# zhouzypaul/fql

Hardware: AMD Instinct MI355X
Metric: FQL gradient-steps/s (batch=256) (higher is better)
Workload: dtype f32

## Files before the change

### fql_amd/csrc/fql_engine.hip

```cpp
#include "../../include/fql_amd.h"
#include "fql_kernels.h"
#include "fql_conv.h"
#include "fql_chain.h"
#include "fql_aux.h"
#include "fql_ifql.h"
#include "fql_rebrac.h"
#include "fql_sac.h"
#include "fql_bc.h"
#include "fql_iql.h"
#include "fql_iqld.h"
#include "fql_cfgrl.h"
#include <hip/hip_ext.h>
#include "fql_aql.h"

#include <algorithm>
#include <cmath>
#include <cstdarg>
#include <cstdio>
#include <cstdlib>
#include <cstring>
#include <map>
#include <memory>
#include <random>
#include <string>
// ... 145 lines not shown
    EulerFinishArgs ef;
    ConvArgs conv;
    PoolArgs pool;
    PoolBwdArgs poolb;
    ConvWgradArgs cw;
    ConvWredArgs cwr;
    EncDzArgs edz;
    ChainArgs chain;
    const ConvWprepTask* wprep_tasks = nullptr;
    int wprep_n = 0;
    int cw_grid = 0;
    int adam_c0 = 0, adam_n = -1;
    int adam_c1 = 0, adam_n1 = 0;
    int adam_polyak = -1;
    float adam_lr = 0.f;
    DevState* adam_st = nullptr;
    bool adam_fin = false;
    int fin_mode = 0;
    Bound k;
    int level = 0;
    int lane = 0;
    std::vector<int> deps;
};

struct Launch {
    OpType type;
    int grid = 0, ntasks = 0;
    size_t lds = 0;
    void* table = nullptr;
    Op op;
    bool pool_fused = false;
    int lane = 0;
    bool tmt2 = false, kbig = false, euler = false;
    double macs = 0.0;
    void *table_w = nullptr, *table_l = nullptr, *table_m = nullptr;
    int n_w = 0, n_l = 0, tile_w = 0, tile_l = 0, tile_m = 0;
    std::vector<GemmTask> dg_tasks;
    std::vector<GemmTask> h_gemm;
    std::vector<WgradTask> h_wgrad;
    std::vector<LnBwdTask> h_ln;
    std::vector<MiscTask> h_misc;
    std::shared_ptr<const SideArgs> ka_side;
    std::vector<int> waits;
    bool record_after = false;
    hipEvent_t ev = nullptr;
};

inline bool ka_tasks_env() {
    const char* e = getenv("FQL_KERNARG_TASKS");
    return !e || atoi(e) != 0;
}
inline bool fused_tail_env() {
    const char* e = getenv("FQL_FUSED_TAIL");
    return !e || atoi(e) != 0;
}
inline std::shared_ptr<const SideArgs> ka_side_args(const Launch& L) {
    const size_t ng = L.h_gemm.size(), nw = L.h_wgrad.size(), nl = L.h_ln.size(), nm = L.h_misc.size();
    if (ng > FQL_KA_GEMM || nw > FQL_KA_WGRAD || nl > FQL_KA_LN || nm > FQL_KA_MISC) return nullptr;
    auto a = std::make_shared<SideArgs>();
    std::memset(a.get(), 0, sizeof(SideArgs));
    SideFront& f = a->f;
    f.tile_w = L.tile_w; f.tile_l = L.tile_l; f.tile_m = L.tile_m; f.tl = -1;
    for (int& v : f.g0) v = FQL_KA_FRONT_PAD;
    for (int& v : f.w0) v = FQL_KA_FRONT_PAD;
    for (int& v : f.l0) v = FQL_KA_FRONT_PAD;
    for (size_t i = 0; i < ng; ++i) { a->g[i] = L.h_gemm[i]; if (i) f.g0[i - 1] = L.h_gemm[i].tile0; }
    for (size_t i = 0; i < nw; ++i) { a->w[i] = L.h_wgrad[i]; if (i) f.w0[i - 1] = L.h_wgrad[i].tile0; }
    for (size_t i = 0; i < nl; ++i) { a->l[i] = L.h_ln[i]; if (i) f.l0[i - 1] = L.h_ln[i].tile0; }
    for (size_t i = 0; i < nm; ++i) a->m[i] = L.h_misc[i];
    return a;
}
struct Program {
    std::vector<Op> ops;
    std::vector<Launch> launches;
    bool lane_used[FQL_LANES] = {};
    hipEvent_t ev_fork = nullptr, ev_join[FQL_LANES] = {};
    hipGraph_t graph = nullptr;
    hipGraphExec_t exec = nullptr;
    int64_t macs = 0;
    AqlProgram aql;
    bool aql_tried = false;
};

template <typename P, typename IssueFn>
void issue_lanes(P& pr, hipStream_t s0, const hipStream_t* ls, bool fork, IssueFn&& issue) {
    auto lazy = [](hipEvent_t& e) { if (!e) HIP_CHECK(hipEventCreateWithFlags(&e, hipEventDisableTiming)); };
    bool side = false;
// ... 210 lines not shown
    size_t n_train = 0, n_total = 0, critic_size = 0;
    float *P = nullptr, *G = nullptr, *Mu = nullptr, *Nu = nullptr;
    std::vector<Leaf> leaves;
    int n_train_leaves = 0;
    AdamChunk* d_chunks = nullptr;
    float* d_partials = nullptr;
    int* d_leaf_range = nullptr;
    int n_chunks = 0;

    DevState* d_state = nullptr;
    SrcDesc* d_src = nullptr;
    SrcDesc h_src_shadow{};
    bool src_valid = false;
    SrcDesc* h_src_ring = nullptr;
    int src_ring_pos = 0;

    int B = 0;
    std::vector<void*> ws_allocs;
    float *in_obs = nullptr, *in_act = nullptr, *in_rew = nullptr, *in_mask = nullptr, *in_nobs = nullptr, *in_nact = nullptr;
    float* in_noise[5] = {nullptr, nullptr, nullptr, nullptr, nullptr};
    int64_t* in_idx = nullptr;
    float *X_os = nullptr, *X_bc = nullptr, *X_eu = nullptr, *X_c1 = nullptr, *X_c2 = nullptr, *X_ct = nullptr;
    float *vel = nullptr, *w_rew = nullptr, *w_mask = nullptr, *w_act = nullptr, *tgt = nullptr;
    float *X_e0 = nullptr, *C0 = nullptr, *Abuf[2] = {nullptr, nullptr}, *Vpart = nullptr;
    bool fused_euler = false;
    bool use_chain = false;
    int fill_lane_full = 1;
    std::vector<float*> wf_bc;
    float *wf_w0 = nullptr, *wf_w4 = nullptr;
    WfragTask* d_wfrag = nullptr;
    int wfrag_n = 0, wfrag_grid = 0;
    const bool ka_tasks = ka_tasks_env();
    const bool fused_tail = fused_tail_env();
    unsigned* d_ticket = nullptr;
    std::vector<void*> chain_allocs;
    bool split_build = false;
    bool wide_tiles = false;
    bool split_ok = false;
    int vp_tiles = 0;
    int num_cus = 0;
    PassBuf p_os, p_os_bwd, p_bc, p_eu, p_c1[2], p_c2[2], p_ct[2];
    Program prog_fwdbwd, prog_opt, prog_loss;
    Program prog_opt_split;
    Program prog_full;
    int mod_chunk0[3] = {0, 0, 0}, mod_chunkn[3] = {0, 0, 0};
    Program prog_split;
    hipGraphExec_t split_exec[4] = {nullptr, nullptr, nullptr, nullptr};
    hipGraph_t split_graph[4] = {nullptr, nullptr, nullptr, nullptr};
    hipEvent_t ev_a = nullptr, ev_b = nullptr, ev_c = nullptr;
    bool split_begun = false;
    bool began = false;
    AqlRuntime aql;
    std::vector<AqlDispatch>* aql_rec = nullptr;
    bool last_update_aql = false;
    bool hip_dirty = true;
    void aql_drain() {
        if (!aql.up) return;
        try { aql.drain(); } catch (const AqlError& e) { throw HipError{e.msg}; }
    }

    float *ds_obs = nullptr, *ds_act = nullptr, *ds_rew = nullptr, *ds_mask = nullptr, *ds_nobs = nullptr;
    float* ds_row = nullptr;
    int64_t ds_size = 0, ds_cap = 0, ds_ptr = 0;
    unsigned char *ds_frames = nullptr, *ds_next_frames = nullptr;
    int64_t* ds_init = nullptr;
    int ds_fs = 0;
// ... 1395 lines not shown
                    for (const Op* o : sel) {
                        Launch L;
                        L.type = (OpType)ty;
                        L.op = *o;
                        L.lane = lane;
                        launch_of[o - pr.ops.data()] = (int)pr.launches.size();
                        pr.launches.push_back(L);
                    }
                    continue;
                }
                Launch L;
                L.type = OP_GEMM;
                L.lane = lane;
                for (const Op* o : sel) launch_of[o - pr.ops.data()] = (int)pr.launches.size();
                L.ntasks = (int)sel.size();
                int tile = 0;
                std::vector<GemmTask> tb;
                for (const Op* o : sel) {
                    GemmTask t = o->gemm;
                    t.wk = (t.N <= 16) ? 4 : 2;
                    t.tmt = 1;
                    t.ntn = (t.N / 16 + (4 / t.wk) - 1) / (4 / t.wk);
                    t.tile0 = tile;
                    tile += (t.M / 16) * t.ntn;
                    if (t.K > 512) L.kbig = true;
                    if (t.flags & (GF_A_EULER0 | GF_HEAD_PART | GF_A_LOSSACT)) L.euler = true;
                    L.lds = std::max(L.lds, ((size_t)16 * (t.K + 4) + 1024 + 1280) * sizeof(float));
                    tb.push_back(t);
                }
                L.table = dalloc(owner, tb.size() * sizeof(GemmTask) / sizeof(float) + 4);
                HIP_CHECK(hipMemcpy(L.table, tb.data(), tb.size() * sizeof(GemmTask), hipMemcpyHostToDevice));
                L.grid = tile;
                L.h_gemm = tb;
                pr.launches.push_back(L);
            }
          }
        }
        auto dump_program = [&]() {
            int cnt[FQL_LANES] = {};
            for (const Launch& L : pr.launches) {
                cnt[L.lane]++;
                int lv = -1;
                for (int oi = 0; oi < (int)pr.ops.size(); ++oi) if (launch_of[oi] == (int)(&L - pr.launches.data())) lv = pr.ops[oi].level;
                fprintf(stderr, "[fql] #%2d level %3d lane %d type %2d ntasks %2d grid %5d waits[", (int)(&L - pr.launches.data()), lv, L.lane, (int)L.type, L.ntasks, L.grid);
                for (int w : L.waits) fprintf(stderr, "%d ", w);
                fprintf(stderr, "] :");
                for (int oi = 0; oi < (int)pr.ops.size(); ++oi) {
                    if (launch_of[oi] != (int)(&L - pr.launches.data())) continue;
                    const Op& o = pr.ops[oi];
                    if (o.type == OP_GEMM || o.type == OP_GEMM64) fprintf(stderr, " g%s(%dx%dx%d%s)", o.type == OP_GEMM64 ? "64" : "16", o.gemm.M, o.gemm.N, o.gemm.K, (o.gemm.flags & GF_TRANS_B) ? "T" : "");
                    else if (o.type == OP_WGRAD) fprintf(stderr, " w(%dx%dx%d)", o.wgrad.M, o.wgrad.Kin, o.wgrad.N);
                    else if (o.type == OP_LNBWD) fprintf(stderr, " ln(%d)", o.ln.M);
                    else fprintf(stderr, " t%d", (int)o.type);
                }
                fprintf(stderr, "\n");
            }
            fprintf(stderr, "[fql] launches per lane:");
            for (int l = 0; l < FQL_LANES; ++l) fprintf(stderr, " %d", cnt[l]);
            fprintf(stderr, "\n");
        };
        for (int oi = 0; oi < (int)pr.ops.size(); ++oi) {
            const Op& o = pr.ops[oi];
            const int li = launch_of[oi];
            if (li < 0) continue;
            double m = 0.0;
            if (o.type == OP_GEMM || o.type == OP_GEMM64 || o.type == OP_HEAD_DGRAD) m = (double)o.gemm.M * o.gemm.N * o.gemm.K;
// ... 50 lines not shown
            if (cost < best) { best = cost; xg = gm; }
        }
        return xg;
    }

    hipEvent_t prof_a = nullptr, prof_b = nullptr;
    template <typename... Pm, typename... A>
    void aql_record(void (*k)(Pm...), dim3 g, dim3 b, size_t l, A&&... a) {
        AqlDispatch d;
        d.fn = (const void*)k;
        d.grid[0] = g.x; d.grid[1] = g.y; d.grid[2] = g.z;
        d.block[0] = b.x; d.block[1] = b.y; d.block[2] = b.z;
        d.lds = (uint32_t)l;
        size_t off = 0;
        auto put = [&](auto v) {
            using T = decltype(v);
            off = (off + alignof(T) - 1) & ~(alignof(T) - 1);
            d.args.resize(off + sizeof(T));
            std::memcpy(d.args.data() + off, &v, sizeof(T));
            off += sizeof(T);
        };
        (put(static_cast<Pm>(a)), ...);
        aql_rec->push_back(std::move(d));
    }
#define FQL_LAUNCH(k, g, b, l, st, ...)                                                          \
    do {                                                                                          \
        if (aql_rec) aql_record(k, g, b, (size_t)(l), __VA_ARGS__);                               \
        else if (prof_a) hipExtLaunchKernelGGL(k, g, b, (std::uint32_t)(l), st, prof_a, prof_b, 0u, __VA_ARGS__); \
        else hipLaunchKernelGGL(k, g, b, l, st, __VA_ARGS__);                                     \
    } while (0)
    void issue(const Launch& L, hipStream_t s, int tl) {
        switch (L.type) {
            case OP_GEMM:
                if (L.euler && L.kbig) FQL_LAUNCH((fql_gemm16_euler_kernel<true>), dim3(L.grid), dim3(FQL_THREADS), L.lds, s, (const GemmTask*)L.table, L.ntasks, tl);
                else if (L.euler) FQL_LAUNCH((fql_gemm16_euler_kernel<false>), dim3(L.grid), dim3(FQL_THREADS), L.lds, s, (const GemmTask*)L.table, L.ntasks, tl);
                else if (L.kbig) FQL_LAUNCH((fql_gemm16_kernel<true>), dim3(L.grid), dim3(FQL_THREADS), L.lds, s, (const GemmTask*)L.table, L.ntasks, tl);
                else FQL_LAUNCH((fql_gemm16_kernel<false>), dim3(L.grid), dim3(FQL_THREADS), L.lds, s, (const GemmTask*)L.table, L.ntasks, tl);
                break;
            case OP_GEMM64:
                if (L.ka_side) {
                    SideArgs a = *L.ka_side; a.f.tl = tl;
                    if (L.tmt2) FQL_LAUNCH(fql_side_big_ka_kernel, dim3(L.grid), dim3(FQL_THREADS), L.lds, s, a);
                    else if (cfg.precision == 2) FQL_LAUNCH(fql_side_split_ka_kernel, dim3(L.grid), dim3(FQL_THREADS), L.lds, s, a);
                    else FQL_LAUNCH(fql_side_ka_kernel, dim3(L.grid), dim3(FQL_THREADS), L.lds, s, a);
                }
                else if (L.tmt2)
                    FQL_LAUNCH(fql_side_big_kernel, dim3(L.grid), dim3(FQL_THREADS), L.lds, s, (const GemmTask*)L.table, L.ntasks,
                                       (const WgradTask*)L.table_w, L.n_w, (const LnBwdTask*)L.table_l, L.n_l, L.tile_w, L.tile_l,
                                       (const MiscTask*)L.table_m, L.tile_m, tl);
                else if (cfg.precision == 2)
                    FQL_LAUNCH(fql_side_split_kernel, dim3(L.grid), dim3(FQL_THREADS), L.lds, s, (const GemmTask*)L.table, L.ntasks,
                                       (const WgradTask*)L.table_w, L.n_w, (const LnBwdTask*)L.table_l, L.n_l, L.tile_w, L.tile_l,
                                       (const MiscTask*)L.table_m, L.tile_m, tl);
                else
                    FQL_LAUNCH(fql_side_kernel, dim3(L.grid), dim3(FQL_THREADS), L.lds, s, (const GemmTask*)L.table, L.ntasks,
                                       (const WgradTask*)L.table_w, L.n_w, (const LnBwdTask*)L.table_l, L.n_l, L.tile_w, L.tile_l,
                                       (const MiscTask*)L.table_m, L.tile_m, tl);
                break;
            case OP_PREP:
                { PrepArgs pa = L.op.prep; pa.tl = tl; FQL_LAUNCH(fql_prep_kernel, dim3((pa.B + 3) / 4), dim3(FQL_THREADS), 0, s, pa); }
                break;
            case OP_EULER_FIN:
                FQL_LAUNCH(fql_euler_finish_kernel, dim3((L.op.ef.M * L.op.ef.ad + FQL_THREADS - 1) / FQL_THREADS), dim3(FQL_THREADS), 0, s, L.op.ef);
                break;
            case OP_LOSS_ACTOR:
                FQL_LAUNCH(fql_loss_actor_kernel, dim3(1), dim3(FQL_THREADS), 0, s, L.op.la);
                break;
// ... 3833 lines not shown
        const int si = code / 100, k = code % 100;
        EncBuf::St& s = b->st[si];
        if (k == 50) {
            const EncStack& st = h->encs[enc].stacks[si];
            std::vector<int32_t> plan{st.conv[0].pool_fused ? 1 : 0};
            for (size_t j = 0; j < st.conv.size(); ++j) {
                const ConvL& c = st.conv[j];
                const int H = j == 0 ? st.H : st.H / 2, W = j == 0 ? st.W : st.W / 2, Ci = pad16c(c.cin);
                const bool u8 = si == 0 && j == 0;
                plan.push_back(u8 ? (h->cfg.precision == 2 ? 1 : 0) : (c.split ? 1 : 0));
                plan.push_back(fql_engine::conv_rows(H, W, Ci, c.cout, false));
                plan.push_back(u8 ? 0 : fql_engine::conv_rows(H, W, c.cout, Ci, false));
                plan.push_back(fql_engine::conv_rows(H, W, Ci, c.cout, true, u8));
            }
            if (bytes > plan.size() * sizeof(int32_t)) return FQL_E_INVALID;
            std::memcpy(out, plan.data(), bytes);
            return FQL_OK;
        }
        if (k == 0) src = s.c0;
        else if (k == 1) src = s.pool;
        else if (k == 4) src = s.arg;
        else if (k % 10 == 2 && (size_t)(k / 10) < s.c1.size()) src = s.c1[k / 10];
        else if (k % 10 == 3 && (size_t)(k / 10) < s.y.size()) src = s.y[k / 10];
    }
    if (!src) return FQL_E_NOTFOUND;
    auto it = b->bytes.find(src);
    if (it == b->bytes.end() || bytes > it->second) return FQL_E_INVALID;
    hipDeviceSynchronize();
    return hipMemcpy(out, src, bytes, hipMemcpyDeviceToHost) == hipSuccess ? FQL_OK : FQL_E_HIP;
}

namespace {
enum { PLAN_K_OTHER = 0, PLAN_K_GEMM16, PLAN_K_GEMM16_KBIG, PLAN_K_GEMM16_EULER, PLAN_K_GEMM16_EULER_KBIG, PLAN_K_SIDE, PLAN_K_SIDE_SPLIT, PLAN_K_SIDE_BIG,
       PLAN_K_CHAIN, PLAN_K_CHAIN_SPLIT };
struct PlanKernel { const void* fn; int entry, H, V; };
template <typename... Pm> const void* plan_fn(void (*k)(Pm...)) { return (const void*)k; }
const std::vector<PlanKernel>& plan_kernels() {
#define FQL_PLAN_CHAIN(HH) \
    {plan_fn(fql_chain_kernel<HH, 0>), PLAN_K_CHAIN, HH, 0}, {plan_fn(fql_chain_kernel<HH, 1>), PLAN_K_CHAIN, HH, 1},                    \
    {plan_fn(fql_chain_kernel<HH, 2>), PLAN_K_CHAIN, HH, 2}, {plan_fn(fql_chain_kernel<HH, 3>), PLAN_K_CHAIN, HH, 3},                    \
    {plan_fn(fql_chain_split_kernel<HH, 0>), PLAN_K_CHAIN_SPLIT, HH, 0}, {plan_fn(fql_chain_split_kernel<HH, 1>), PLAN_K_CHAIN_SPLIT, HH, 1}, \
    {plan_fn(fql_chain_split_kernel<HH, 2>), PLAN_K_CHAIN_SPLIT, HH, 2}
    static const std::vector<PlanKernel> t = {
        {plan_fn(fql_gemm16_kernel<false>), PLAN_K_GEMM16, 0, 0}, {plan_fn(fql_gemm16_kernel<true>), PLAN_K_GEMM16_KBIG, 0, 0},
        {plan_fn(fql_gemm16_euler_kernel<false>), PLAN_K_GEMM16_EULER, 0, 0}, {plan_fn(fql_gemm16_euler_kernel<true>), PLAN_K_GEMM16_EULER_KBIG, 0, 0},
        {plan_fn(fql_side_kernel), PLAN_K_SIDE, 0, 0}, {plan_fn(fql_side_split_kernel), PLAN_K_SIDE_SPLIT, 0, 0},
        {plan_fn(fql_side_big_kernel), PLAN_K_SIDE_BIG, 0, 0}, FQL_PLAN_CHAIN(256), FQL_PLAN_CHAIN(512),
        {plan_fn(fql_side_ka_kernel), PLAN_K_SIDE, 0, 0}, {plan_fn(fql_side_split_ka_kernel), PLAN_K_SIDE_SPLIT, 0, 0},
        {plan_fn(fql_side_big_ka_kernel), PLAN_K_SIDE_BIG, 0, 0}};
#undef FQL_PLAN_CHAIN
    return t;
}
}
extern "C" int fql_debug_plan(fql_handle h, void* out, size_t bytes) {
    if (!h || (bytes && !out) || bytes % sizeof(int32_t)) return FQL_E_INVALID;
    if (h->visual || !h->prog_full.exec || h->prog_full.launches.empty()) return FQL_E_STATE;
    try {
        const Program& pr = h->prog_full;
        const std::vector<AqlDispatch> rec = h->record_dispatches(pr);
        std::vector<int32_t> plan{0, (int32_t)pr.launches.size()};
        for (size_t i = 0; i < pr.launches.size(); ++i) {
            const Launch& L = pr.launches[i];
            const AqlDispatch& d = rec[i];
            PlanKernel k{d.fn, PLAN_K_OTHER, 0, 0};
            for (const PlanKernel& c : plan_kernels()) if (c.fn == d.fn) k = c;
            const bool table = L.type == OP_GEMM || L.type == OP_GEMM64;
            const bool chain = L.type == OP_CHAIN;
            if (chain != (k.entry == PLAN_K_CHAIN || k.entry == PLAN_K_CHAIN_SPLIT)) throw HipError{"internal: a chain launch records an unknown kernel"};
            if (table == (k.entry == PLAN_K_OTHER || chain)) throw HipError{"internal: a GEMM launch records an unknown kernel"};
            plan.insert(plan.end(), {(int32_t)i, L.lane, (int32_t)L.type, (int32_t)(d.grid[0] * d.grid[1] * d.grid[2]), k.entry,
                                     table ? (int32_t)L.h_gemm.size() : 0, table ? (int32_t)L.h_wgrad.size() : 0, table ? (int32_t)L.h_ln.size() : 0,
                                     chain ? 1 : 0});
            if (table) {
                for (const GemmTask& t : L.h_gemm) plan.insert(plan.end(), {t.M, t.N, t.K, (L.type == OP_GEMM ? 16 : 32) * t.tmt, t.wk, t.xg});
                for (const WgradTask& t : L.h_wgrad) plan.insert(plan.end(), {t.M, t.Kin, t.N, k.entry == PLAN_K_SIDE_SPLIT ? 1 : 0});
                for (const LnBwdTask& t : L.h_ln) plan.push_back(t.M);
            }
            if (chain) {
                ChainArgs ca;
                if (d.args.size() < sizeof(ChainArgs)) throw HipError{"internal: a chain launch records no ChainArgs"};
                std::memcpy(&ca, d.args.data(), sizeof(ChainArgs));
                plan.insert(plan.end(), {ca.M, k.H, k.V, ca.xg, k.entry == PLAN_K_CHAIN_SPLIT ? 1 : 0});
// ... 153 lines not shown
            F.ev = nullptr; F.waits.clear();
            F.ka_side = nullptr;
            std::vector<WfragTask> h_wf;
            std::vector<const void*> tg, tw, tl, tm;
            std::vector<int> ng, nw, nl, nm, sg, sw, sl, sm;
            int cg = 0, cw = 0, cl = 0, cm = 0, ntot = 0;
            for (int k = 0; k < K; ++k) {
                const Launch& L = m[k]->prog_full.launches[li];
                if (L0.type == OP_WFRAG) {
                    tg.push_back(m[k]->d_wfrag); ng.push_back(m[k]->wfrag_n); sg.push_back(cg); cg += m[k]->wfrag_grid; ntot += m[k]->wfrag_n;
                } else if (L0.type == OP_GEMM64) {
                    tg.push_back(L.table); ng.push_back(L.ntasks); sg.push_back(cg); cg += L.tile_w;
                    tw.push_back(L.table_w); nw.push_back(L.n_w); sw.push_back(cw); cw += L.tile_l - L.tile_w;
                    tl.push_back(L.table_l); nl.push_back(L.n_l); sl.push_back(cl); cl += L.tile_m - L.tile_l;
                    tm.push_back(L.table_m); nm.push_back(L.grid - L.tile_m); sm.push_back(0); cm += L.grid - L.tile_m;
                } else {
                    tg.push_back(L.table); ng.push_back(L.ntasks); sg.push_back(cg); cg += L.grid; ntot += L.ntasks;
                }
            }
            if (L0.type == OP_WFRAG) {
                F.table = fuse<WfragTask>(tg, ng, sg, h_wf); F.ntasks = ntot; F.grid = cg;
            } else if (L0.type == OP_GEMM64) {
                F.table = fuse<GemmTask>(tg, ng, sg, F.h_gemm);
                F.table_w = fuse<WgradTask>(tw, nw, sw, F.h_wgrad);
                F.table_l = fuse<LnBwdTask>(tl, nl, sl, F.h_ln);
                F.table_m = fuse<MiscTask>(tm, nm, sm, F.h_misc, false);
                F.ntasks = F.n_w = F.n_l = 0;
                for (int k = 0; k < K; ++k) { F.ntasks += ng[k]; F.n_w += nw[k]; F.n_l += nl[k]; }
                F.tile_w = cg; F.tile_l = cg + cw; F.tile_m = cg + cw + cl; F.grid = F.tile_m + cm;
                if (m[0]->ka_tasks) F.ka_side = ka_side_args(F);
            } else {
                F.table = fuse<GemmTask>(tg, ng, sg, F.h_gemm);
                F.ntasks = ntot; F.grid = cg;
            }
            G.L = F;
            return G;
        }
        auto it = multi_entries().find(rec[0].fn);
        if (it == multi_entries().end()) invalid("agent groups: launch %d (op type %d) has no multi-instance kernel", li, (int)L0.type);
        std::vector<uint8_t> args;
        for (int k = 0; k < K; ++k) {
            if (rec[k].args.size() != it->second.arg_bytes) invalid("internal: launch %d records %zu argument bytes, its struct has %zu", li, rec[k].args.size(), it->second.arg_bytes);
            args.insert(args.end(), rec[k].args.begin(), rec[k].args.end());
        }
        G.multi = it->second.launch;
        G.grid = dim3(rec[0].grid[0], K);
        G.block = dim3(rec[0].block[0], rec[0].block[1], rec[0].block[2]);
        G.lds = rec[0].lds;
        G.args = upload(args.data(), args.size());
        return G;
    }

    void issue(GLaunch& G, hipStream_t s) {
        if (!G.table) { G.multi(G.grid, G.block, G.lds, s, G.args); return; }
        if (G.L.type == OP_WFRAG) hipLaunchKernelGGL(fql_wfrag_kernel, dim3(G.L.grid), dim3(FQL_THREADS), 0, s, (const WfragTask*)G.L.table, G.L.ntasks, -1);
        else m[0]->issue(G.L, s, -1);
    }

    void capture() {
        capture_graph(lanes[0], [&] { issue_lanes(*this, lanes[0], lanes, true, [&](GLaunch& G, hipStream_t s) { issue(G, s); }); }, graph, exec);
    }

    void release() {
        if (lanes[0]) hipStreamSynchronize(lanes[0]);
        if (last == hipStreamLegacy) hipDeviceSynchronize();
        if (ev_done) hipEventSynchronize(ev_done);
// ... 1 lines not shown
        if (exec) hipGraphExecDestroy(exec);
        if (graph) hipGraphDestroy(graph);
        destroy_lane_events(*this);
        for (hipEvent_t e : {ev_in, ev_done}) if (e) hipEventDestroy(e);
        for (void* p : allocs) hipFree(p);
        if (d_idx) hipFree(d_idx);
        for (hipStream_t s : lanes) if (s) hipStreamDestroy(s);
    }
};

namespace {
void group_check(const fql_handle* members, int k) {
    if (!members || k <= 0) invalid("fql_group_create: members must be a non-empty array (k = %d)", k);
    for (int i = 0; i < k; ++i) {
        fql_handle h = members[i];
        if (!h) invalid("fql_group_create: member %d is NULL", i);
        for (int j = 0; j < i; ++j) if (members[j] == h) invalid("fql_group_create: member %d appears twice", i);
        if (h->group) invalid("fql_group_create: member %d already belongs to a group", i);
        if (h->visual) invalid("fql_group_create: member %d has an encoder (groups take state agents only)", i);
        if (h->cfg.precision != 0) invalid("fql_group_create: member %d has precision %d (groups take fp32 members only)", i, h->cfg.precision);
        if (h->began) invalid("fql_group_create: member %d is between fql_update_begin and fql_update_end", i);
        require_graph(h->prog_full);
        fql_config a = h->cfg, b = members[0]->cfg;
        a.alpha = b.alpha = 0.f;
        a.batch_size = b.batch_size = 0;
        if (std::memcmp(&a, &b, sizeof a) != 0)
            invalid("fql_group_create: member %d's config differs from member 0's in more than seed and alpha", i);
        if (h->B != members[0]->B) invalid("fql_group_create: member %d has batch size %d, member 0 has %d", i, h->B, members[0]->B);
        const Program& p = h->prog_full, &p0 = members[0]->prog_full;
        if (p.launches.size() != p0.launches.size()) invalid("fql_group_create: member %d's update has %zu launches, member 0's %zu", i, p.launches.size(), p0.launches.size());
        for (size_t li = 0; li < p.launches.size(); ++li) {
            const Launch &L = p.launches[li], &L0 = p0.launches[li];
            if (L.type != L0.type || L.lane != L0.lane || L.grid != L0.grid || L.waits != L0.waits || L.tmt2 != L0.tmt2 ||
                L.kbig != L0.kbig || L.euler != L0.euler || L.record_after != L0.record_after || L.lds != L0.lds)
                invalid("fql_group_create: launch %zu of member %d differs from member 0's (type %d/%d, lane %d/%d, grid %d/%d)", li, i, (int)L.type,
                        (int)L0.type, L.lane, L0.lane, L.grid, L0.grid);
            if (L.type == OP_WFRAG && h->wfrag_grid != members[0]->wfrag_grid) invalid("fql_group_create: member %d's weight-copy launch differs", i);
        }
    }
}
}

extern "C" {

int fql_group_create(const fql_handle* members, int k, fql_group* out) {
    if (!out) { g_create_error = "fql_group_create: out must not be NULL"; return FQL_E_INVALID; }
    *out = nullptr;
    for (int i = 0; members && i < k; ++i)
        if (members[i] && members[i]->kind != AgentKind::FQL) {
            g_create_error = "fql_group_create: member " + std::to_string(i) + " is " + members[i]->desc().label + " (groups take FQL agents only)";
            return FQL_E_STATE;
        }
    auto* g = new fql_group_s();
    try {
        group_check(members, k);
        g->m.assign(members, members + k);
        g->K = k;
        g->B = members[0]->B;
        for (fql_handle h : g->m) { h->aql_drain(); HIP_CHECK(hipStreamSynchronize(h->stream)); }
        std::vector<std::vector<AqlDispatch>> rec;
        for (fql_handle h : g->m) rec.push_back(h->record_dispatches(h->prog_full));
        const size_t n = g->m[0]->prog_full.launches.size();
        for (size_t li = 0; li < n; ++li)
            for (int i = 1; i < k; ++i) {
                const AqlDispatch &a = rec[i][li], &b = rec[0][li];
                if (a.fn != b.fn || std::memcmp(a.grid, b.grid, sizeof a.grid) || std::memcmp(a.block, b.block, sizeof a.block) || a.lds != b.lds)
                    invalid("fql_group_create: launch %zu of member %d runs another kernel or shape than member 0's", li, i);
// ... 95 lines not shown
```

### fql_amd/csrc/fql_kernels.h

```cpp
#pragma once
#include <hip/hip_runtime.h>
#include <stdint.h>

typedef float f32x4 __attribute__((ext_vector_type(4)));

#define FQL_GAS __attribute__((address_space(1)))
__device__ __forceinline__ float ldg(const float* p) { return *(const FQL_GAS float*)p; }
__device__ __forceinline__ f32x4 ldg4(const float* p) { return *(const FQL_GAS f32x4*)p; }
__device__ __forceinline__ void stg(float* p, float v) { *(FQL_GAS float*)p = v; }
__device__ __forceinline__ void stg4(float* p, f32x4 v) { *(FQL_GAS f32x4*)p = v; }

#define FQL_THREADS 256

struct FastDiv {
    unsigned m;
    int d;
    __device__ __forceinline__ explicit FastDiv(int dd) : m(dd > 1 ? 0xFFFFFFFFu / (unsigned)dd + 1u : 0u), d(dd) {}
    __device__ __forceinline__ FastDiv(int dd, unsigned long long max_x) : m(dd > 1 && max_x * (unsigned long long)dd < (1ull << 32) ? 0xFFFFFFFFu / (unsigned)dd + 1u : 0u), d(dd) {}
    __device__ __forceinline__ int div(int x) const { return m ? (int)__umulhi((unsigned)x, m) : (d == 1 ? x : (int)((unsigned)x / (unsigned)d)); }
    __device__ __forceinline__ void divmod(int x, int& q, int& r) const { q = div(x); r = x - q * d; }
};

__device__ __forceinline__ float frcp(int d) { return __builtin_amdgcn_rcpf((float)d); }
__device__ __forceinline__ int sdiv(int x, float rd) { return (int)(((float)x + 0.5f) * rd); }
// ... 736 lines not shown
    }
    }
#ifdef FQL_STAMPS
    STAMP();
    if (lane == 0 && wave == 0 && T.aux) {
        unsigned long long* d = reinterpret_cast<unsigned long long*>(T.aux) + (size_t)blockIdx.x * 8;
        for (int i = 0; i < nst; ++i) d[i] = stamp[i];
    }
#endif
}

#ifndef FQL_GEMM_WAVES
#define FQL_GEMM_WAVES 1
#endif
template <bool KBIG>
__global__ __launch_bounds__(FQL_THREADS, FQL_GEMM_WAVES) void fql_gemm16_kernel(const GemmTask* __restrict__ tasks, int ntasks, int tl) {
    extern __shared__ __attribute__((aligned(16))) float lds[];
    tl_enter(tl);
    const GemmTask& T = tasks[find_task(tasks, ntasks, blockIdx.x)];
    if (T.K <= 128) gemm16_body<2, 1, false>(T, lds);
    else if (!KBIG || T.K <= 512) gemm16_body<8, 1, false>(T, lds);
    else gemm16_body<16, 1, false>(T, lds);
    tl_exit(tl);
}
template <bool KBIG>
__global__ __launch_bounds__(FQL_THREADS) void fql_gemm16_euler_kernel(const GemmTask* __restrict__ tasks, int ntasks, int tl) {
    extern __shared__ __attribute__((aligned(16))) float lds[];
    tl_enter(tl);
    const GemmTask& T = tasks[find_task(tasks, ntasks, blockIdx.x)];
    if (T.K <= 128) gemm16_body<2, 1, true>(T, lds);
    else if (!KBIG || T.K <= 512) gemm16_body<8, 1, true>(T, lds);
    else gemm16_body<16, 1, true>(T, lds);
    tl_exit(tl);
}

#define G64_S 68
template <int NR>
__device__ __forceinline__ void ln_fold_partials(const float* __restrict__ partials, int row_first, int ntin, float (&sum)[NR], float (&sumsq)[NR]) {
    const int rs = (2 * ntin + 3) & ~3;
    const int nf4 = (ntin + 1) >> 1;
#pragma unroll
    for (int i = 0; i < NR; ++i) { sum[i] = 0.f; sumsq[i] = 0.f; }
    for (int base = 0; base < nf4; base += 4) {
        f32x4 pv[NR][4];
#pragma unroll
        for (int i = 0; i < NR; ++i) {
            const float* pp = partials + (size_t)(row_first + 16 * i) * rs;
#pragma unroll
            for (int t = 0; t < 4; ++t) pv[i][t] = ldg4(pp + 4 * min(base + t, nf4 - 1));
        }
#pragma unroll
        for (int i = 0; i < NR; ++i)
#pragma unroll
            for (int t = 0; t < 4; ++t) {
                if (2 * (base + t) < ntin) { sum[i] += pv[i][t][0]; sumsq[i] += pv[i][t][1]; }
                if (2 * (base + t) + 1 < ntin) { sum[i] += pv[i][t][2]; sumsq[i] += pv[i][t][3]; }
            }
    }
}

template <bool transb, int RI>
__device__ __forceinline__ void gemm64_body(const GemmTask& T, float* lds) {
    constexpr int TM = 32 * RI;
    float* As = lds;
    float* Bs = lds + 2 * TM * G64_S;
    float* part = Bs + 2 * 64 * G64_S;
// ... 1499 lines not shown
```

Measured before the change: 2987.

## Add specialized head16 kernel for N=16 head GEMMs with kernarg task records

Adds a dedicated kernel for the 16-column output head GEMMs (K up to 512), selected by default for eligible launches. Each workgroup splits K across four waves that hold operands in registers, does an optional fused LayerNorm, runs MFMA, and reduces the partial results through LDS. Task records are passed in kernel arguments rather than a device table. The aim is to cut the latency of these small, latency-bound GEMMs, at the cost of more specialized code and an env switch to fall back.

New measurement: 2860. 0.958x the previous value.

```diff
diff --git a/experiments/head_bench.hip b/experiments/head_bench.hip
--- /dev/null
+++ b/experiments/head_bench.hip
@@ -0,0 +1,81 @@
+#include "../fql_amd/csrc/fql_kernels.h"
+#include <chrono>
+#include <cstdio>
+#include <cstdlib>
+#include <cstring>
+#include <vector>
+#define CK(x) do { hipError_t e = (x); if (e != hipSuccess) { printf("%s: %s\n", #x, hipGetErrorString(e)); exit(1); } } while (0)
+int main(int argc, char** argv) {
+    const int preset = argc > 1 ? atoi(argv[1]) : 0;
+    const int K = 512, nt = preset == 0 ? 4 : 2;
+    const int Ms[4] = {preset == 0 ? 256 : 768, 256, 256, 256};
+    const int flags = preset == 0 ? (GF_BIAS | GF_A_LN | GF_LN_WRITE) : GF_BIAS;
+    hipStream_t s; CK(hipStreamCreateWithFlags(&s, hipStreamNonBlocking));
+    size_t rows = 0;
+    for (int i = 0; i < nt; ++i) rows += Ms[i];
+    float *A, *XN, *W, *b, *C, *stats;
+    CK(hipMalloc(&A, rows * K * 4)); CK(hipMalloc(&XN, rows * K * 4)); CK(hipMalloc(&W, (size_t)4 * K * 16 * 4)); CK(hipMalloc(&b, 2048 * 4));
+    CK(hipMalloc(&C, rows * 16 * 4)); CK(hipMalloc(&stats, rows * 2 * 4));
+    std::vector<float> hw((size_t)4 * K * 16), ha(rows * K), ones(2048, 1.0f);
+    for (size_t i = 0; i < hw.size(); ++i) hw[i] = ((float)((i * 2654435761u) >> 8 & 0xFFFF) / 65536.0f - 0.5f) * 0.08f;
+    for (size_t i = 0; i < ha.size(); ++i) ha[i] = ((float)((i * 40503u) & 0xFFFF) / 65536.0f - 0.5f);
+    CK(hipMemcpy(W, hw.data(), hw.size() * 4, hipMemcpyHostToDevice)); CK(hipMemcpy(A, ha.data(), ha.size() * 4, hipMemcpyHostToDevice));
+    CK(hipMemcpy(b, ones.data(), 2048 * 4, hipMemcpyHostToDevice));
+    unsigned long long* stamps; CK(hipMalloc(&stamps, 8 * 256 * 8)); CK(hipMemset(stamps, 0, 8 * 256 * 8));
+    std::vector<GemmTask> h(nt);
+    Head16Args ha16;
+    std::memset(&ha16, 0, sizeof ha16);
+    for (int& v : ha16.f.t0) v = FQL_KA_FRONT_PAD;
+    ha16.f.tl = -1;
+#ifdef FQL_HEAD_STAMPS
+    ha16.f.stamps64 = stamps;
+#endif
+    int grid = 0;
+    size_t r0 = 0;
+    for (int i = 0; i < nt; ++i) {
+        GemmTask t{};
+        t.A = A + r0 * K; t.lda = K; t.B = W + (size_t)i * K * 16; t.ldb = 16; t.bias = b; t.C = C + r0 * 16; t.ldc = 16;
+        t.M = Ms[i]; t.N = 16; t.K = K; t.flags = flags; t.ntn = 1; t.wk = 4; t.tmt = 1; t.tile0 = grid;
+        t.ln_g = b + 512; t.ln_b = b + 1024; t.ln_width = K; t.ln_xout = XN + r0 * K; t.ln_stats = stats + r0 * 2;
+        h[i] = t;
+        HeadTask& d = ha16.t[i];
+        d.A = t.A; d.B = t.B; d.bias = t.bias; d.C = t.C; d.ln_g = t.ln_g; d.ln_b = t.ln_b; d.ln_xout = t.ln_xout; d.ln_stats = t.ln_stats;
+        d.M = t.M; d.K = t.K; d.lda = t.lda; d.ldb = t.ldb; d.ldc = t.ldc; d.ln_width = t.ln_width; d.flags = t.flags; d.tile0 = t.tile0;
+        if (i) ha16.f.t0[i - 1] = grid;
+        grid += Ms[i] / 16;
+        r0 += Ms[i];
+    }
+    GemmTask* tb; CK(hipMalloc(&tb, nt * sizeof(GemmTask)));
+    CK(hipMemcpy(tb, h.data(), nt * sizeof(GemmTask), hipMemcpyHostToDevice));
+    const size_t lds = ((size_t)16 * (K + 4) + 1024 + 1280) * sizeof(float);
+    for (int which = 0; which < 2; ++which) {
+        hipGraph_t g; hipGraphExec_t ge;
+        CK(hipStreamBeginCapture(s, hipStreamCaptureModeThreadLocal));
+        for (int i = 0; i < 48; ++i)
+            if (which) hipLaunchKernelGGL(fql_head16_kernel, dim3(grid), dim3(FQL_THREADS), 0, s, ha16);
+            else hipLaunchKernelGGL((fql_gemm16_kernel<false>), dim3(grid), dim3(FQL_THREADS), lds, s, (const GemmTask*)tb, nt, -1);
+        CK(hipStreamEndCapture(s, &g)); CK(hipGraphInstantiate(&ge, g, nullptr, nullptr, 0));
+        for (int i = 0; i < 10; ++i) CK(hipGraphLaunch(ge, s));
+        CK(hipStreamSynchronize(s));
+        auto t0 = std::chrono::high_resolution_clock::now();
+        for (int i = 0; i < 30; ++i) CK(hipGraphLaunch(ge, s));
+        CK(hipStreamSynchronize(s));
+        const double us = std::chrono::duration<double, std::micro>(std::chrono::high_resolution_clock::now() - t0).count() / (30 * 48);
+        printf("%s preset=%d tasks=%d grid=%d : %.2f us per launch\n", which ? "fql_head16_kernel" : "fql_gemm16_kernel<false>", preset, nt, grid, us);
+        CK(hipGraphExecDestroy(ge)); CK(hipGraphDestroy(g));
+    }
+#ifdef FQL_HEAD_STAMPS
+    std::vector<unsigned long long> st((size_t)8 * grid);
+    CK(hipMemcpy(st.data(), stamps, st.size() * 8, hipMemcpyDeviceToHost));
+    double ph[5] = {0, 0, 0, 0, 0};
+    unsigned long long first = ~0ull, last = 0;
+    for (int w = 0; w < grid; ++w) {
+        for (int i = 0; i < 5; ++i) ph[i] += (double)(st[w * 8 + i + 1] - st[w * 8 + i]) / 100.0;
+        first = first < st[w * 8] ? first : st[w * 8];
+        last = last > st[w * 8 + 5] ? last : st[w * 8 + 5];
+    }
+    printf("   fql_head16_kernel in-kernel (us, mean over WGs): operand loads %.2f | LayerNorm %.2f | MFMA %.2f | part exchange %.2f | epilogue %.2f ; first-entry..last-exit %.2f\n",
+           ph[0] / grid, ph[1] / grid, ph[2] / grid, ph[3] / grid, ph[4] / grid, (double)(last - first) / 100.0);
+#endif
+    return 0;
+}
diff --git a/experiments/heads_check.py b/experiments/heads_check.py
--- /dev/null
+++ b/experiments/heads_check.py
@@ -0,0 +1,226 @@
+#!/usr/bin/env python3
+import os
+import sys
+
+import numpy as np
+import pytest
+import torch
+
+sys.path.insert(0, os.path.dirname(os.path.dirname(os.path.abspath(__file__))))
+
+from oracle import fql_oracle as O
+from tests.test_gpu_group import _assert_same_state as assert_same_group_state, _setup as group_setup
+from tests.util import (K_GEMM16, OP_GEMM, assert_same_state, assert_step_matches, assert_total_loss_matches, leaf_dict, make_problem,
+                        randomize_params, read_plan)
+
+pytestmark = pytest.mark.gpu
+SWITCH = 'FQL_HEAD16'
+K_HEAD16 = 10
+HEAD_CAP = 4
+
+
+def _with_switch_off(make):
+    old = os.environ.get(SWITCH)
+    os.environ[SWITCH] = '0'
+    try:
+        return make()
+    finally:
+        if old is None:
+            del os.environ[SWITCH]
+        else:
+            os.environ[SWITCH] = old
+
+
+def _problem(od, ad, B, hidden, seed=3, **kw):
+    import fql_amd
+    cfg, ds, batch, noise = make_problem(od, ad, B, hidden, seed=seed, **kw)
+
+    def make():
+        a = fql_amd.FQLAgent.create(1, batch['observations'][:1], batch['actions'][:1], cfg)
+        a.set_params(randomize_params(a.get_params(), seed + 1, scale=0.05 if max(hidden) >= 512 else 0.1))
+        a.upload_dataset(ds)
+        return a
+    return make, cfg, ds, batch, noise
+
+
+def _head_launches(plan):
+    return [L for L in plan if L['type'] == OP_GEMM and L['gemm'] and all(t['N'] == 16 for t in L['gemm'])]
+
+
+def _eligible(L):
+    return len(L['gemm']) <= HEAD_CAP and all(t['K'] % 128 == 0 and t['K'] <= 512 and t['M'] % 16 == 0 for t in L['gemm'])
+
+
+def _assert_paths(a, b, strict=False):
+    pa, pb = read_plan(a), read_plan(b)
+    heads = _head_launches(pa)
+    assert heads, 'no launch of 16-column heads in the plan'
+    for L in pa:
+        if L['kernel'] == K_HEAD16:
+            assert L in heads and _eligible(L), L
+            assert all(t['rows'] == 16 and t['wk'] == 4 for t in L['gemm']), L
+        elif L in heads and _eligible(L):
+            assert len(L['gemm']) == 1 and not strict, L
+    assert all(L['kernel'] != K_HEAD16 for L in pb)
+    assert all(L['kernel'] == K_GEMM16 for L in _head_launches(pb))
+    return pa, pb
+
+
+def _three_updates(agents, ds, B, ad, streams=None):
+    rng = np.random.default_rng(5)
+    for step in range(3):
+        idxs = rng.integers(0, len(ds['observations']), size=B)
+        nz = O.make_noise(B, ad, 40 + step)
+        for i, x in enumerate(agents):
+            kw = dict(stream=streams[i].cuda_stream) if streams and streams[i] is not None else {}
+            x.update_from_dataset(B, idxs=idxs, noise=nz, **kw)
+        for i, x in enumerate(agents):
+            x.synchronize()
+            if streams and streams[i] is not None:
+                streams[i].synchronize()
+        infos = [x.read_info() for x in agents]
+        assert len(infos[0]) == 13 and all(i == infos[0] for i in infos[1:]), (step, infos)
+    for x in agents[1:]:
+        assert_same_state(agents[0], x)
+
+
+CASES = {
+    'h128x2_b16': (29, 8, 16, (128, 128), {}),
+    'h256x2_b48': (29, 8, 48, (256, 256), {}),
+    'h384x2_b32': (29, 8, 32, (384, 384), {}),
+    'flagship': (29, 8, 256, (512,) * 4, {}),
+    'act1': (29, 1, 32, (128, 128), {}),
+    'act16': (29, 16, 32, (128, 128), {}),
+    'q_min': (29, 8, 32, (128, 128), dict(q_agg='min')),
+    'q_mean': (29, 8, 32, (128, 128), dict(q_agg='mean')),
+    'norm_q': (29, 8, 32, (128, 128), dict(normalize_q_loss=True)),
+    'actor_ln': (29, 8, 32, (256, 256), dict(actor_layer_norm=True)),
+    'bf16x3': (29, 8, 64, (256,) * 4, dict(precision='bf16x3')),
+}
+
+
+@pytest.mark.parametrize('cid', list(CASES))
+def test_head_kernel_equals_generic_kernel_bitwise(cid):
+    od, ad, B, hidden, kw = CASES[cid]
+    make, cfg, ds, batch, noise = _problem(od, ad, B, hidden, **kw)
+    a, b = make(), _with_switch_off(make)
+    pa, _ = _assert_paths(a, b)
+    on_head = [t for L in pa if L['kernel'] == K_HEAD16 for t in L['gemm']]
+    assert {t['K'] for t in on_head} == {hidden[-1]}
+    assert {t['M'] for t in on_head} >= {B, 3 * B}
+    if cid == 'h256x2_b48':
+        assert 144 in {t['M'] for t in on_head}
+    _three_updates([a, b], ds, B, ad)
+
+
+def test_act17_actor_heads_stay_on_the_generic_kernel():
+    od, ad, B, hidden = 29, 17, 32, (128, 128)
+    make, cfg, ds, batch, noise = _problem(od, ad, B, hidden)
+    a, b = make(), _with_switch_off(make)
+    pa, _ = _assert_paths(a, b)
+    wide = [L for L in pa if L['type'] == OP_GEMM and any((t['N'], t['K']) == (32, 128) for t in L['gemm'])]
+    assert wide and all(L['kernel'] == K_GEMM16 for L in wide)
+    assert any(L['kernel'] == K_HEAD16 for L in pa)
+    _three_updates([a, b], ds, B, ad)
+
+
+def test_captured_graph_on_a_callers_stream_against_the_engines_queues():
+    import torch
+    od, ad, B, hidden = 29, 8, 64, (256,) * 4
+    make, cfg, ds, batch, noise = _problem(od, ad, B, hidden)
+    a, b, c = make(), make(), _with_switch_off(make)
+    _assert_paths(a, c)
+    st = torch.cuda.Stream()
+    _three_updates([a, b, c], ds, B, ad, streams=[None, st, None])
+    assert a.synchronize() == 'aql' and b.synchronize() == 'graph'
+
+
+@pytest.mark.parametrize('K', [2, 3])
+def test_group_members_equal_their_standalone_twins(K):
+    B, H = 64, 128
+    _, _, _, _, group, twins = group_setup(K, B, H)
+    for m, t in zip(group.members, twins):
+        pm, pt = read_plan(m), read_plan(t)
+        assert pm == pt and any(L['kernel'] == K_HEAD16 for L in pm)
+        assert all((L['kernel'] == K_HEAD16) == _eligible(L) for L in _head_launches(pm))
+    for _ in range(5):
+        group.update_from_dataset()
+        for t in twins:
+            t.update_from_dataset(B)
+    group.synchronize()
+    for i, (m, t) in enumerate(zip(group.members, twins)):
+        assert_same_group_state(m, t, f'member {i}')
+    group.close()
+
+
+def test_total_loss_and_sample_actions_leave_the_state_alone():
+    od, ad, B, hidden = 29, 8, 32, (128, 128)
+    make, cfg, ds, batch, noise = _problem(od, ad, B, hidden)
+    a, b = make(), _with_switch_off(make)
+    _assert_paths(a, b)
+    rng = np.random.default_rng(9)
+    obs = rng.standard_normal((37, od)).astype(np.float32)
+    z = rng.standard_normal((37, ad)).astype(np.float32)
+
+    def probes():
+        outs = []
+        for x in (a, b):
+            before = leaf_dict(x.get_params())
+            loss, info = x.total_loss(batch, noise=noise)
+            act = x.sample_actions(obs, noises=z)
+            after = leaf_dict(x.get_params())
+            for k in before:
+                np.testing.assert_array_equal(before[k], after[k], err_msg=k)
+            outs.append((loss, info, act))
+        (la, ia, aa), (lb, ib, ab) = outs
+        assert la == lb and ia == ib
+        np.testing.assert_array_equal(aa, ab)
+    probes()
+    _three_updates([a, b], ds, B, ad)
+    probes()
+
+
+@pytest.mark.parametrize('cid', ['h128x2_b16', 'flagship'])
+def test_update_on_the_head_kernel_matches_the_fp64_oracle(cid):
+    od, ad, B, hidden, kw = CASES[cid]
+    import fql_amd
+    cfg, ds, batch, noise = make_problem(od, ad, B, hidden, seed=3, **kw)
+    agent = fql_amd.FQLAgent.create(0, batch['observations'][:1], batch['actions'][:1], cfg)
+    params = randomize_params(agent.get_params(), seed=5, scale=0.05 if max(hidden) >= 512 else 0.1)
+    agent.set_params(params)
+    assert any(L['kernel'] == K_HEAD16 for L in read_plan(agent))
+    ref = O.OracleFQL(params, dict(cfg), od, ad, np.float64)
+    assert_total_loss_matches(agent, ref, params, batch, noise)
+    worst = assert_step_matches(agent, ref, cfg, batch, noise)
+    print(f'{cid}: worst relative gradient error {worst[0]:.3e} ({worst[1]})')
+
+
+def test_plan_of_the_flagship_program():
+    od, ad, B, hidden, kw = CASES['flagship']
+    make, cfg, ds, batch, noise = _problem(od, ad, B, hidden, **kw)
+    a, b = make(), _with_switch_off(make)
+    pa, pb = _assert_paths(a, b, strict=True)
+    heads = _head_launches(pa)
+    assert heads and all(L['kernel'] == K_HEAD16 for L in heads)
+    assert sum(len(L['gemm']) for L in heads) >= 8
+    na, nb = len(pa), len(pb)
+    print(f'launches per update: default {na}, FQL_HEAD16=0 {nb}')
+    assert a.stats()['launches_per_update'] == na and b.stats()['launches_per_update'] == nb
+    assert na == nb == 80
+    assert a.stats()['macs_per_update'] == b.stats()['macs_per_update']
+
+
+if __name__ == '__main__':
+    torch.zeros(1, device='cuda')
+    for cid in CASES:
+        test_head_kernel_equals_generic_kernel_bitwise(cid)
+        print('ok bitwise', cid, flush=True)
+    test_act17_actor_heads_stay_on_the_generic_kernel()
+    test_captured_graph_on_a_callers_stream_against_the_engines_queues()
+    for K in (2, 3):
+        test_group_members_equal_their_standalone_twins(K)
+    test_total_loss_and_sample_actions_leave_the_state_alone()
+    for cid in ('h128x2_b16', 'flagship'):
+        test_update_on_the_head_kernel_matches_the_fp64_oracle(cid)
+    test_plan_of_the_flagship_program()
+    print('heads_check: all cases ok')
diff --git a/fql_amd/csrc/fql_engine.hip b/fql_amd/csrc/fql_engine.hip
--- a/fql_amd/csrc/fql_engine.hip
+++ b/fql_amd/csrc/fql_engine.hip
@@ -201,6 +201,7 @@
     bool pool_fused = false;
     int lane = 0;
     bool tmt2 = false, kbig = false, euler = false;
+    bool head = false;
     double macs = 0.0;
     void *table_w = nullptr, *table_l = nullptr, *table_m = nullptr;
     int n_w = 0, n_l = 0, tile_w = 0, tile_l = 0, tile_m = 0;
@@ -222,6 +223,31 @@
 inline bool fused_tail_env() {
     const char* e = getenv("FQL_FUSED_TAIL");
     return !e || atoi(e) != 0;
+}
+inline bool head16_env() {
+    const char* e = getenv("FQL_HEAD16");
+    return !e || atoi(e) != 0;
+}
+inline bool head16_ok(const GemmTask& t) {
+    constexpr int allowed = GF_BIAS | GF_A_LN | GF_LN_WRITE | GF_OS_SCATTER | GF_CLIP_OUT;
+    return t.N == 16 && !(t.flags & GF_TRANS_B) && t.K % 128 == 0 && t.K <= 512 && t.M % 16 == 0 && !(t.flags & ~allowed);
+}
+inline Head16Args head16_args(const std::vector<GemmTask>& tb, int tl) {
+    Head16Args a;
+    std::memset(&a, 0, sizeof a);
+    for (int& v : a.f.t0) v = FQL_KA_FRONT_PAD;
+    a.f.tl = tl;
+    for (size_t i = 0; i < tb.size() && i < FQL_KA_HEAD; ++i) {
+        const GemmTask& t = tb[i];
+        HeadTask& h = a.t[i];
+        h.A = t.A; h.B = t.B; h.bias = t.bias; h.C = t.C;
+        h.ln_g = t.ln_g; h.ln_b = t.ln_b; h.ln_xout = t.ln_xout; h.ln_stats = t.ln_stats;
+        h.aux = t.aux; h.aux2 = t.aux2;
+        h.M = t.M; h.K = t.K; h.lda = t.lda; h.ldb = t.ldb; h.ldc = t.ldc; h.ln_width = t.ln_width; h.flags = t.flags; h.tile0 = t.tile0;
+        h.i0 = t.i0; h.i1 = t.i1; h.i2 = t.i2;
+        if (i) a.f.t0[i - 1] = t.tile0;
+    }
+    return a;
 }
 inline std::shared_ptr<const SideArgs> ka_side_args(const Launch& L) {
     const size_t ng = L.h_gemm.size(), nw = L.h_wgrad.size(), nl = L.h_ln.size(), nm = L.h_misc.size();
@@ -498,6 +524,7 @@
     int wfrag_n = 0, wfrag_grid = 0;
     const bool ka_tasks = ka_tasks_env();
     const bool fused_tail = fused_tail_env();
+    const bool head16 = head16_env();
     unsigned* d_ticket = nullptr;
     std::vector<void*> chain_allocs;
     bool split_build = false;
@@ -1959,6 +1986,7 @@
                 HIP_CHECK(hipMemcpy(L.table, tb.data(), tb.size() * sizeof(GemmTask), hipMemcpyHostToDevice));
                 L.grid = tile;
                 L.h_gemm = tb;
+                L.head = head16 && kind == AgentKind::FQL && tb.size() <= FQL_KA_HEAD && std::all_of(tb.begin(), tb.end(), head16_ok);
                 pr.launches.push_back(L);
             }
           }
@@ -2075,7 +2103,8 @@
     void issue(const Launch& L, hipStream_t s, int tl) {
         switch (L.type) {
             case OP_GEMM:
-                if (L.euler && L.kbig) FQL_LAUNCH((fql_gemm16_euler_kernel<true>), dim3(L.grid), dim3(FQL_THREADS), L.lds, s, (const GemmTask*)L.table, L.ntasks, tl);
+                if (L.head) FQL_LAUNCH(fql_head16_kernel, dim3(L.grid), dim3(FQL_THREADS), 0, s, head16_args(L.h_gemm, tl));
+                else if (L.euler && L.kbig) FQL_LAUNCH((fql_gemm16_euler_kernel<true>), dim3(L.grid), dim3(FQL_THREADS), L.lds, s, (const GemmTask*)L.table, L.ntasks, tl);
                 else if (L.euler) FQL_LAUNCH((fql_gemm16_euler_kernel<false>), dim3(L.grid), dim3(FQL_THREADS), L.lds, s, (const GemmTask*)L.table, L.ntasks, tl);
                 else if (L.kbig) FQL_LAUNCH((fql_gemm16_kernel<true>), dim3(L.grid), dim3(FQL_THREADS), L.lds, s, (const GemmTask*)L.table, L.ntasks, tl);
                 else FQL_LAUNCH((fql_gemm16_kernel<false>), dim3(L.grid), dim3(FQL_THREADS), L.lds, s, (const GemmTask*)L.table, L.ntasks, tl);
@@ -5975,7 +6004,7 @@
 
 namespace {
 enum { PLAN_K_OTHER = 0, PLAN_K_GEMM16, PLAN_K_GEMM16_KBIG, PLAN_K_GEMM16_EULER, PLAN_K_GEMM16_EULER_KBIG, PLAN_K_SIDE, PLAN_K_SIDE_SPLIT, PLAN_K_SIDE_BIG,
-       PLAN_K_CHAIN, PLAN_K_CHAIN_SPLIT };
+       PLAN_K_CHAIN, PLAN_K_CHAIN_SPLIT, PLAN_K_HEAD16 };
 struct PlanKernel { const void* fn; int entry, H, V; };
 template <typename... Pm> const void* plan_fn(void (*k)(Pm...)) { return (const void*)k; }
 const std::vector<PlanKernel>& plan_kernels() {
@@ -5990,7 +6019,8 @@
         {plan_fn(fql_side_kernel), PLAN_K_SIDE, 0, 0}, {plan_fn(fql_side_split_kernel), PLAN_K_SIDE_SPLIT, 0, 0},
         {plan_fn(fql_side_big_kernel), PLAN_K_SIDE_BIG, 0, 0}, FQL_PLAN_CHAIN(256), FQL_PLAN_CHAIN(512),
         {plan_fn(fql_side_ka_kernel), PLAN_K_SIDE, 0, 0}, {plan_fn(fql_side_split_ka_kernel), PLAN_K_SIDE_SPLIT, 0, 0},
-        {plan_fn(fql_side_big_ka_kernel), PLAN_K_SIDE_BIG, 0, 0}};
+        {plan_fn(fql_side_big_ka_kernel), PLAN_K_SIDE_BIG, 0, 0},
+        {plan_fn(fql_head16_kernel), PLAN_K_HEAD16, 0, 0}};
 #undef FQL_PLAN_CHAIN
     return t;
 }
@@ -6210,6 +6240,7 @@
             } else {
                 F.table = fuse<GemmTask>(tg, ng, sg, F.h_gemm);
                 F.ntasks = ntot; F.grid = cg;
+                F.head = L0.head && ntot <= FQL_KA_HEAD;
             }
             G.L = F;
             return G;
@@ -6277,7 +6308,7 @@
         for (size_t li = 0; li < p.launches.size(); ++li) {
             const Launch &L = p.launches[li], &L0 = p0.launches[li];
             if (L.type != L0.type || L.lane != L0.lane || L.grid != L0.grid || L.waits != L0.waits || L.tmt2 != L0.tmt2 ||
-                L.kbig != L0.kbig || L.euler != L0.euler || L.record_after != L0.record_after || L.lds != L0.lds)
+                L.kbig != L0.kbig || L.euler != L0.euler || L.head != L0.head || L.record_after != L0.record_after || L.lds != L0.lds)
                 invalid("fql_group_create: launch %zu of member %d differs from member 0's (type %d/%d, lane %d/%d, grid %d/%d)", li, i, (int)L.type,
                         (int)L0.type, L.lane, L0.lane, L.grid, L0.grid);
             if (L.type == OP_WFRAG && h->wfrag_grid != members[0]->wfrag_grid) invalid("fql_group_create: member %d's weight-copy launch differs", i);
diff --git a/fql_amd/csrc/fql_kernels.h b/fql_amd/csrc/fql_kernels.h
--- a/fql_amd/csrc/fql_kernels.h
+++ b/fql_amd/csrc/fql_kernels.h
@@ -792,6 +792,192 @@
     else if (!KBIG || T.K <= 512) gemm16_body<8, 1, true>(T, lds);
     else gemm16_body<16, 1, true>(T, lds);
     tl_exit(tl);
+}
+
+struct HeadTask {
+    const float* A;
+    const float* B;
+    const float* bias;
+    float* C;
+    const float* ln_g;
+    const float* ln_b;
+    float* ln_xout;
+    float* ln_stats;
+    float* aux;
+    float* aux2;
+    int M, K, lda, ldb, ldc, ln_width, flags, tile0;
+    int i0, i1, i2;
+    int pad;
+};
+#define FQL_KA_HEAD 4
+struct HeadFront {
+    int t0[FQL_KA_HEAD - 1];
+    int tl;
+#ifdef FQL_HEAD_STAMPS
+    unsigned long long* stamps64;
+    int pad[10];
+#else
+    int pad[12];
+#endif
+};
+struct Head16Args {
+    HeadFront f;
+    HeadTask t[FQL_KA_HEAD];
+};
+static_assert(sizeof(HeadFront) == 64 && sizeof(HeadTask) == 128, "the front is one 16-dword load, a record two");
+static_assert(sizeof(Head16Args) <= FQL_KA_LIMIT, "Head16Args and the hidden block must fit the 4 KB of a launch's arguments");
+__device__ __forceinline__ void gemm_mma_chunk(f32x4& acc, f32x4& acc2, const float (&b)[32], const f32x4 (&a)[8]) {
+#pragma unroll
+    for (int g = 0; g < 8; g += 2) {
+#pragma unroll
+        for (int s = 0; s < 4; ++s) {
+            acc = __builtin_amdgcn_mfma_f32_16x16x4f32(a[g][s], b[4 * g + s], acc, 0, 0, 0);
+            acc2 = __builtin_amdgcn_mfma_f32_16x16x4f32(a[g + 1][s], b[4 * g + 4 + s], acc2, 0, 0, 0);
+        }
+    }
+}
+#define FQL_HEAD_S(K) ((K) + 16)
+template <int NG>
+__device__ __forceinline__ void head16_body(const HeadTask& T, int local, float* tile, float* red, float* st, unsigned long long* dbg) {
+    constexpr int K = 64 * NG, KQ = 16 * NG, S = FQL_HEAD_S(K);
+    const int tid = threadIdx.x, kp = tid >> 6, lane = tid & 63, c = lane & 15, q = lane >> 4;
+#ifdef FQL_HEAD_STAMPS
+    unsigned long long stamp[8];
+    int nst = 0;
+#define HSTAMP() do { __builtin_amdgcn_s_waitcnt(0); stamp[nst++] = __builtin_amdgcn_s_memrealtime(); } while (0)
+#else
+#define HSTAMP() do {} while (0)
+#endif
+    HSTAMP();
+    const int row0 = local * 16, flags = T.flags;
+    const int k0 = kp * KQ + 4 * q;
+    const int er = lane >> 2, ec = lane & 3;
+    f32x4 a[NG];
+    float b[4 * NG];
+    {
+        const float* __restrict__ ap = T.A + (size_t)(row0 + c) * T.lda + k0;
+#pragma unroll
+        for (int g = 0; g < NG; ++g) a[g] = ldg4(ap + 16 * g);
+        const float* __restrict__ bp = T.B + (size_t)k0 * T.ldb + c;
+#pragma unroll
+        for (int g = 0; g < NG; ++g)
+#pragma unroll
+            for (int s = 0; s < 4; ++s) b[4 * g + s] = ldg(bp + (size_t)(16 * g + s) * T.ldb);
+    }
+    f32x4 bias4 = {0.f, 0.f, 0.f, 0.f};
+    if (kp == 0 && (flags & GF_BIAS)) bias4 = ldg4(T.bias + 4 * ec);
+    HSTAMP();
+    if (flags & GF_A_LN) {
+        f32x4 gm[NG], bt[NG];
+#pragma unroll
+        for (int g = 0; g < NG; ++g) { gm[g] = ldg4(T.ln_g + k0 + 16 * g); bt[g] = ldg4(T.ln_b + k0 + 16 * g); }
+        const int width = T.ln_width;
+        const bool wr = (flags & GF_LN_WRITE) != 0;
+#pragma unroll
+        for (int g = 0; g < NG; ++g) *reinterpret_cast<f32x4*>(&tile[c * S + k0 + 16 * g]) = a[g];
+        __syncthreads();
+        {
+            const int r = tid >> 4, j = tid & 15;
+            float s = 0.f, s2 = 0.f;
+#pragma unroll
+            for (int i = 0; i < K / 16; ++i) {
+                const float x = tile[r * S + j + 16 * i];
+                if (j + 16 * i < width) { s += x; s2 = fmaf(x, x, s2); }
+            }
+#pragma unroll
+            for (int o = 1; o < 16; o <<= 1) {
+                s += __shfl_xor(s, o);
+                s2 += __shfl_xor(s2, o);
+            }
+            const float inv = 1.0f / (float)width;
+            const float mean = s * inv;
+            const float var = fmaxf(0.0f, fmaf(s2, inv, -(mean * mean)));
+            const float rstd = 1.0f / sqrtf(var + 1e-6f);
+            if (j == 0) {
+                st[2 * r] = mean; st[2 * r + 1] = rstd;
+                if (wr) {
+                    stg(T.ln_stats + 2 * (row0 + r), mean);
+                    stg(T.ln_stats + 2 * (row0 + r) + 1, rstd);
+                }
+            }
+        }
+        __syncthreads();
+        const float mean = st[2 * c], rstd = st[2 * c + 1];
+#pragma unroll
+        for (int g = 0; g < NG; ++g) {
+            f32x4 v;
+#pragma unroll
+            for (int e = 0; e < 4; ++e) v[e] = (k0 + 16 * g + e < width) ? fmaf((a[g][e] - mean) * rstd, gm[g][e], bt[g][e]) : 0.f;
+            a[g] = v;
+            if (wr) stg4(T.ln_xout + (size_t)(row0 + c) * T.lda + k0 + 16 * g, v);
+        }
+    }
+    HSTAMP();
+    f32x4 acc = {0.f, 0.f, 0.f, 0.f};
+    if constexpr (NG == 8) {
+        f32x4 acc2 = {0.f, 0.f, 0.f, 0.f};
+        gemm_mma_chunk(acc, acc2, b, a);
+        acc += acc2;
+    } else {
+#pragma unroll
+        for (int g = 0; g < NG; ++g)
+#pragma unroll
+            for (int s = 0; s < 4; ++s) acc = __builtin_amdgcn_mfma_f32_16x16x4f32(a[g][s], b[4 * g + s], acc, 0, 0, 0);
+    }
+    HSTAMP();
+    *reinterpret_cast<f32x4*>(&red[(kp * 64 + lane) * 4]) = acc;
+    __syncthreads();
+    if (kp != 0) return;
+    HSTAMP();
+    const int row = row0 + er;
+    f32x4 v;
+#pragma unroll
+    for (int e = 0; e < 4; ++e) {
+        const int o = (16 * (er >> 2) + 4 * ec + e) * 4 + (er & 3);
+        float x = red[o];
+        x += red[256 + o];
+        x += red[512 + o];
+        x += red[768 + o];
+        x += bias4[e];
+        v[e] = (flags & GF_CLIP_OUT) ? clip1(x) : x;
+    }
+    stg4(T.C + (size_t)row * T.ldc + 4 * ec, v);
+    if (flags & GF_OS_SCATTER) {
+        const int B3 = T.M / 3;
+        float* dst = row < B3 ? T.aux + (size_t)row * T.i0 + T.i1 : row < 2 * B3 ? T.aux2 + (size_t)(row - B3) * T.i0 + T.i1 : nullptr;
+        if (dst) {
+#pragma unroll
+            for (int e = 0; e < 4; ++e)
+                if (4 * ec + e < T.i2) stg(dst + 4 * ec + e, clip1(v[e]));
+        }
+    }
+#ifdef FQL_HEAD_STAMPS
+    HSTAMP();
+    if (lane == 0 && dbg) {
+        unsigned long long* d = dbg + (size_t)blockIdx.x * 8;
+        for (int i = 0; i < nst; ++i) d[i] = stamp[i];
+    }
+#endif
+#undef HSTAMP
+}
+__global__ __launch_bounds__(FQL_THREADS) void fql_head16_kernel(const Head16Args) {
+    __shared__ __attribute__((aligned(16))) float tile[16 * FQL_HEAD_S(512)];
+    __shared__ __attribute__((aligned(16))) float red[4 * 64 * 4];
+    __shared__ float st[32];
+    const HeadFront F = ka_load<HeadFront>(ka_base());
+    tl_enter(F.tl);
+    const HeadTask T = ka_load<HeadTask>(ka_base() + offsetof(Head16Args, t) + (size_t)find_front(F.t0, (int)blockIdx.x) * sizeof(HeadTask));
+    const int local = (int)blockIdx.x - T.tile0;
+#ifdef FQL_HEAD_STAMPS
+    unsigned long long* dbg = F.stamps64;
+#else
+    unsigned long long* dbg = nullptr;
+#endif
+    if (T.K == 512) head16_body<8>(T, local, tile, red, st, dbg);
+    else if (T.K == 384) head16_body<6>(T, local, tile, red, st, dbg);
+    else if (T.K == 256) head16_body<4>(T, local, tile, red, st, dbg);
+    else head16_body<2>(T, local, tile, red, st, dbg);
+    tl_exit(F.tl);
 }
 
 #define G64_S 68
```
